# duylebkHCM/EyeDiseaseSegmentation

Measured on NVIDIA B200. Metric: IDRiD-size (2848x4288) fundus images/s, 4 lesion models, sliding-window + 8-view D4 TTA + AUC-PR, higher is better.
Workload: dtype bf16

## Files before the change

eyediseasesegmentation_b200/csrc/conv3x3_wide_sm100.cu:

```cuda
#include "tc_ptx.cuh"
#include <algorithm>
#include <cstdlib>
#include <cstring>
#include <mutex>

namespace eds {

constexpr int kWideThreads = 320;
constexpr int kWideStagesMax = 4;
constexpr int kWideRows = 8, kWideSlabCols = 32, kWideOutCols = 30, kWideSlabRows = kWideRows + 2;

struct WideParams {
    CUtensorMap a_map;
    CUtensorMap a_map1;
    int k_split;
    CUtensorMap b_map;
    CUtensorMap y_map;
    const float* bias;
    const __nv_bfloat16* residual;
    __nv_bfloat16* y;
    int C, block_k, k_chunks, bn;
    int N, H, W, relu;
    int tiles_w, tiles_h, total_tiles;
    int stages, atom_bytes, a_slab_bytes, b_box_bytes, stage_bytes, tmem_cols;
    int b_resident, b_region_bytes;
    int staged, staging_off;
    uint32_t idesc, desc_hi;
};

__device__ __forceinline__ void wide_mbar_arrive(uint64_t* bar) {
    asm volatile("mbarrier.arrive.shared::cta.b64 _, [%0];" ::"r"(smem_u32(bar)) : "memory");
}

__global__ void __launch_bounds__(kWideThreads, 1)
conv3x3_wide_kernel(const __grid_constant__ WideParams p) {
    extern __shared__ uint8_t smem_raw[];
    uint8_t* smem = reinterpret_cast<uint8_t*>((reinterpret_cast<uintptr_t>(smem_raw) + 1023) & ~(uintptr_t)1023);
    uint8_t* ring = smem + p.b_region_bytes;
    uint64_t* full_bar = reinterpret_cast<uint64_t*>(ring + (size_t)p.stages * p.stage_bytes);
    uint64_t* empty_bar = full_bar + kWideStagesMax;
    uint64_t* tmem_full_bar = empty_bar + kWideStagesMax;
    uint64_t* tmem_empty_bar = tmem_full_bar + 2;
    uint64_t* b_bar = tmem_empty_bar + 2;
    uint32_t* tmem_slot = reinterpret_cast<uint32_t*>(b_bar + 1);
    float* s_bias = reinterpret_cast<float*>(full_bar + 16);
    if (threadIdx.x < (unsigned)p.bn) s_bias[threadIdx.x] = p.bias ? __ldg(p.bias + threadIdx.x) : 0.f;

    const int warp = threadIdx.x >> 5, lane = threadIdx.x & 31;
    if (warp == 0 && lane == 0) {
        prefetch_tmap(&p.a_map);
        prefetch_tmap(&p.a_map1);
        prefetch_tmap(&p.b_map);
        for (int s = 0; s < p.stages; ++s) {
            mbar_init(&full_bar[s], 1);
            mbar_init(&empty_bar[s], 1);
        }
        for (int m = 0; m < 2; ++m) {
            mbar_init(&tmem_full_bar[m], 1);
            mbar_init(&tmem_empty_bar[m], 4);
        }
        mbar_init(b_bar, 1);
        asm volatile("fence.mbarrier_init.release.cluster;" ::: "memory");
        asm volatile("fence.proxy.async.shared::cta;" ::: "memory");
    }
    if (warp == 1) tmem_alloc(tmem_slot, (uint32_t)p.tmem_cols);
    tc_fence_before();
    __syncthreads();
    tc_fence_after();
    const uint32_t tmem_base = *tmem_slot;
    const uint32_t n3 = 3u * (uint32_t)p.bn;

    if (warp == 0) {
        if (lane == 0) {
            int stage = 0;
            uint32_t phase = 0;
            const uint32_t a_tx = (uint32_t)(kWideSlabRows * 4 * p.atom_bytes), b_tx = (uint32_t)(9 * p.bn * p.block_k * 2);
            const uint32_t tx = p.b_resident ? a_tx : a_tx + b_tx;
            if (p.b_resident) {
                mbar_arrive_expect_tx(b_bar, b_tx * (uint32_t)p.k_chunks);
                for (int kc = 0; kc < p.k_chunks; ++kc)
                    for (int tap = 0; tap < 9; ++tap)
                        tma_load_2d(smem + (size_t)(kc * 9 + tap) * p.b_box_bytes, &p.b_map, b_bar,
                                    tap * p.C + kc * p.block_k, 0);
            }
            for (int tile = blockIdx.x; tile < p.total_tiles; tile += gridDim.x) {
                const int tw = tile % p.tiles_w;
                const int t2 = tile / p.tiles_w;
                const int th = t2 % p.tiles_h;
                const int n = t2 / p.tiles_h;
                const int w0 = tw * kWideOutCols, h0 = th * kWideRows;
                for (int kc = 0; kc < p.k_chunks; ++kc) {
                    mbar_wait(&empty_bar[stage], phase ^ 1u);
                    mbar_arrive_expect_tx(&full_bar[stage], tx);
                    uint8_t* sa = ring + (size_t)stage * p.stage_bytes;
                    uint8_t* sb = sa + p.a_slab_bytes;
                    if (kc < p.k_split)
                        tma_load_4d(sa, &p.a_map, &full_bar[stage], kc * p.block_k, w0 - 1, h0 - 1, n);
                    else
                        tma_load_4d(sa, &p.a_map1, &full_bar[stage], (kc - p.k_split) * p.block_k, w0 - 1, h0 - 1, n);
                    if (!p.b_resident)
                        for (int tap = 0; tap < 9; ++tap)
                            tma_load_2d(sb + tap * p.b_box_bytes, &p.b_map, &full_bar[stage], tap * p.C + kc * p.block_k, 0);
                    if (++stage == p.stages) { stage = 0; phase ^= 1u; }
                }
            }
        }
    } else if (warp == 1) {
        int stage = 0;
        uint32_t phase = 0;
        const uint32_t lo0 = desc_lo(smem_u32(ring)), blo0 = desc_lo(smem_u32(smem));
        const uint32_t stage16 = (uint32_t)p.stage_bytes >> 4, slab16 = (uint32_t)p.a_slab_bytes >> 4;
        const uint32_t bchunk16 = 9u * ((uint32_t)p.b_box_bytes >> 4);
        if (p.b_resident) mbar_wait(b_bar, 0);
        const uint32_t atom16 = (uint32_t)p.atom_bytes >> 4, brow16 = 3u * ((uint32_t)p.b_box_bytes >> 4);
        const uint32_t dhi_w = p.desc_hi, idesc = p.idesc;
        const int k_steps = p.block_k / 16;
        int t = 0;
        for (int tile = blockIdx.x; tile < p.total_tiles; tile += gridDim.x, ++t) {
            const uint32_t empty_parity = (uint32_t)((t & 1) ^ 1);
            for (int kc = 0; kc < p.k_chunks; ++kc) {
                mbar_wait(&full_bar[stage], phase);
                const uint32_t a_st = lo0 + (uint32_t)stage * stage16;
                const uint32_t b_st = p.b_resident ? blo0 + (uint32_t)kc * bchunk16 : a_st + slab16;
#pragma unroll
                for (int m = 0; m < 2; ++m) {
                    if (kc == 0) mbar_wait(&tmem_empty_bar[m], empty_parity);
                    tc_fence_after();
                    if (elect_one()) {
                        const uint32_t d = tmem_base + (uint32_t)m * n3;
#pragma unroll
                        for (int dhi = 0; dhi < 3; ++dhi) {
                            const uint32_t a_lo = a_st + (uint32_t)(m * 16 + dhi * 4) * atom16;
                            const uint32_t b_lo = b_st + (uint32_t)dhi * brow16;
                            for (int ks = 0; ks < k_steps; ++ks)
                                umma_bf16_lohi(d, a_lo + 2u * ks, b_lo + 2u * ks, dhi_w, idesc,
                                               (kc > 0 || dhi > 0 || ks > 0) ? 1u : 0u);
                        }
                    }
                    __syncwarp();
                    if (kc == p.k_chunks - 1) {
                        if (elect_one()) umma_commit(&tmem_full_bar[m]);
                        __syncwarp();
                    }
                }
                if (elect_one()) umma_commit(&empty_bar[stage]);
                __syncwarp();
                if (++stage == p.stages) { stage = 0; phase ^= 1u; }
            }
        }
    } else {
        const int q = warp & 3;
        const int m = (warp - 2) >> 2;
        const int bn = p.bn;
        uint8_t* stg = smem + p.staging_off + (size_t)(warp - 2) * 4096;
        const int pos = lane - 1;
        int t = 0;
        for (int tile = blockIdx.x; tile < p.total_tiles; tile += gridDim.x, ++t) {
            const int tw = tile % p.tiles_w;
            const int t2 = tile / p.tiles_w;
            const int th = t2 % p.tiles_h;
            const int n = t2 / p.tiles_h;
            const int ow = tw * kWideOutCols - 1 + lane;
            const bool col_ok = lane >= 1 && lane <= kWideOutCols && ow < p.W;
            {
                mbar_wait(&tmem_full_bar[m], (uint32_t)(t & 1));
                tc_fence_after();
                const int oh = th * kWideRows + m * 4 + q;
                const bool valid = col_ok && oh < p.H;
                const int64_t off = (((int64_t)n * p.H + oh) * p.W + ow) * bn;
                const uint32_t taddr = tmem_base + ((uint32_t)(q * 32) << 16) + (uint32_t)m * n3;
                if (p.staged) {
                    if (lane == 0) asm volatile("cp.async.bulk.wait_group.read 0;" ::: "memory");
                    __syncwarp();
                }
                for (int c = 0; c < bn; c += 16) {
                    uint32_t rl[16], rc[16], rr[16];
                    tmem_ld16_nowait(taddr + (uint32_t)c, rl);
                    tmem_ld16_nowait(taddr + (uint32_t)(bn + c), rc);
                    tmem_ld16_nowait(taddr + (uint32_t)(2 * bn + c), rr);
                    tmem_ld_wait();
                    float v[16];
#pragma unroll
                    for (int i = 0; i < 16; ++i) {
                        const float l = __shfl_up_sync(0xffffffffu, __uint_as_float(rl[i]), 1);
                        const float r = __shfl_down_sync(0xffffffffu, __uint_as_float(rr[i]), 1);
                        v[i] = (l + __uint_as_float(rc[i])) + r;
                    }
                    if (valid || (p.staged && pos >= 0 && pos < kWideOutCols)) {
                        {
                            const float4* b4 = reinterpret_cast<const float4*>(s_bias + c);
#pragma unroll
                            for (int i = 0; i < 4; ++i) {
                                const float4 b = b4[i];
                                v[4 * i] += b.x; v[4 * i + 1] += b.y; v[4 * i + 2] += b.z; v[4 * i + 3] += b.w;
                            }
                        }
                        if (p.residual && valid) {
                            float r0[8], r1[8];
                            Vec8<__nv_bfloat16>::ld(p.residual + off + c, r0);
                            Vec8<__nv_bfloat16>::ld(p.residual + off + c + 8, r1);
#pragma unroll
                            for (int i = 0; i < 8; ++i) { v[i] += r0[i]; v[8 + i] += r1[i]; }
                        }
                        if (p.relu) {
#pragma unroll
                            for (int i = 0; i < 16; ++i) v[i] = fmaxf(v[i], 0.f);
                        }
                        float o0[8], o1[8];
#pragma unroll
                        for (int i = 0; i < 8; ++i) { o0[i] = v[i]; o1[i] = v[8 + i]; }
                        if (p.staged) {
                            const uint32_t j = (uint32_t)c >> 3, sw = (uint32_t)pos & 7u;
                            Vec8<__nv_bfloat16>::st(reinterpret_cast<__nv_bfloat16*>(stg + pos * 128 + ((j ^ sw) << 4)), o0);
                            Vec8<__nv_bfloat16>::st(reinterpret_cast<__nv_bfloat16*>(stg + pos * 128 + (((j + 1) ^ sw) << 4)), o1);
                        } else {
                            Vec8<__nv_bfloat16>::st(p.y + off + c, o0);
                            Vec8<__nv_bfloat16>::st(p.y + off + c + 8, o1);
                        }
                    }
                }
                if (p.staged) {
                    asm volatile("fence.proxy.async.shared::cta;" ::: "memory");
                    __syncwarp();
                    if (lane == 0 && oh < p.H) {
                        asm volatile(
                            "cp.async.bulk.tensor.4d.global.shared::cta.bulk_group [%0, {%2, %3, %4, %5}], [%1];"
                            ::"l"(&p.y_map), "r"(smem_u32(stg)), "r"(0), "r"(tw * kWideOutCols), "r"(oh), "r"(n)
                            : "memory");
                        asm volatile("cp.async.bulk.commit_group;" ::: "memory");
                    }
                }
                tc_fence_before();
                __syncwarp();
                if (lane == 0) wide_mbar_arrive(&tmem_empty_bar[m]);
            }
        }
        if (p.staged && lane == 0) asm volatile("cp.async.bulk.wait_group 0;" ::: "memory");
    }

    tc_fence_before();
    __syncthreads();
    if (warp == 1) tmem_dealloc(tmem_base, (uint32_t)p.tmem_cols);
}

static PerDevice g_wide_once;
static int g_wide_sms = 148;

static int wide_init() {
    return g_wide_once.run([](int dev) {
        cudaError_t e = cudaFuncSetAttribute(conv3x3_wide_kernel, cudaFuncAttributeMaxDynamicSharedMemorySize, 227 * 1024);
        if (e != cudaSuccess) {
            set_error("conv3x3_wide: cannot opt in to 227 KB shared memory: %s", cudaGetErrorString(e));
            return (int)EDS_ERR_CUDA;
        }
        int sms = 0;
        if (cudaDeviceGetAttribute(&sms, cudaDevAttrMultiProcessorCount, dev) == cudaSuccess && sms > 0) g_wide_sms = sms;
        return (int)EDS_OK;
    });
}

}

using namespace eds;

extern "C" int eds_conv3x3_wide_supported(int C, int Cout, int R, int S, int stride, int pad) {
    return R == 3 && S == 3 && stride == 1 && pad == 1 && C >= 16 && C % 16 == 0 && Cout >= 16 && Cout % 16 == 0 &&
           Cout <= 64;
}

static int wide_launch(const void* x, int C0, const void* x1, int C1, int N, int H, int W, const void* w,
                       const float* bias, int Cout, int relu, const void* residual, void* y, void* stream) {
    const int C = C0 + C1;
    EDS_REQUIRE(x && w && y, "conv3x3_wide: null pointer");
    EDS_REQUIRE(C0 >= 16 && C0 % 16 == 0 && C1 >= 0 && C1 % 16 == 0 && (x1 != nullptr) == (C1 > 0),
                "conv3x3_wide: C0=%d C1=%d must be multiples of 16", C0, C1);
    EDS_REQUIRE(N > 0 && H > 0 && W > 0, "conv3x3_wide: bad shape N=%d H=%d W=%d", N, H, W);
    EDS_REQUIRE(eds_conv3x3_wide_supported(C, Cout, 3, 3, 1, 1),
                "conv3x3_wide: C=%d Cout=%d outside the supported range (multiples of 16, Cout <= 64)", C, Cout);
    EDS_REQUIRE((((uintptr_t)x | (uintptr_t)x1 | (uintptr_t)w | (uintptr_t)y | (uintptr_t)residual | (uintptr_t)bias) &
                 15) == 0, "conv3x3_wide: pointers must be 16-byte aligned");
    if (int rc = igemm_init()) return rc;
    if (int rc = wide_init()) return rc;

    WideParams p;
    memset(&p, 0, sizeof(p));
    p.bias = bias;
    p.residual = (const __nv_bfloat16*)residual;
    p.y = (__nv_bfloat16*)y;
    p.C = C;
    p.block_k = ((C0 | C1) % 64 == 0) ? 64 : ((C0 | C1) % 32 == 0 ? 32 : 16);
    if (const char* bk = getenv("EDS_WIDE_BK")) {
        const int v = atoi(bk);
        if ((v == 32 || v == 16) && (C0 | C1) % v == 0) p.block_k = std::min(p.block_k, v);
    }
    p.k_chunks = C / p.block_k;
    p.k_split = C0 / p.block_k;
    p.bn = Cout;
    p.N = N; p.H = H; p.W = W; p.relu = relu;
    p.tiles_w = ceil_div(W, kWideOutCols);
    p.tiles_h = ceil_div(H, kWideRows);
    const int64_t total = (int64_t)p.tiles_w * p.tiles_h * N;
    EDS_REQUIRE(total < (1ll << 31), "conv3x3_wide: too many tiles");
    p.total_tiles = (int)total;

    const CUtensorMapSwizzle swz = p.block_k == 64 ? CU_TENSOR_MAP_SWIZZLE_128B
                                  : p.block_k == 32 ? CU_TENSOR_MAP_SWIZZLE_64B : CU_TENSOR_MAP_SWIZZLE_32B;
    const uint32_t layout = p.block_k == 64 ? 2u : (p.block_k == 32 ? 4u : 6u);
    p.atom_bytes = 8 * p.block_k * 2;
    const uint32_t sbo = (uint32_t)p.atom_bytes >> 4;
    p.desc_hi = sbo | (1u << 14) | (layout << 29);
    p.idesc = (1u << 4) | (1u << 7) | (1u << 10) | ((uint32_t)((3 * p.bn) >> 3) << 17) | ((uint32_t)(128 >> 4) << 24);
    p.a_slab_bytes = (kWideSlabRows * 4 * p.atom_bytes + 1023) & ~1023;
    p.b_box_bytes = p.bn * p.block_k * 2;
    const int barrier_bytes = 128 + 64 * 4;
    const int budget = 227 * 1024 - 1024 - barrier_bytes;
    const int b_all = p.k_chunks * 9 * p.b_box_bytes;
    static const bool no_resident = getenv("EDS_WIDE_RESIDENT") && atoi(getenv("EDS_WIDE_RESIDENT")) == 0;
    p.b_resident = !no_resident && b_all + 3 * p.a_slab_bytes <= budget;
    p.b_region_bytes = p.b_resident ? ((b_all + 1023) & ~1023) : 0;
    p.stage_bytes = p.b_resident ? p.a_slab_bytes : ((p.a_slab_bytes + 9 * p.b_box_bytes + 1023) & ~1023);
    p.stages = std::min(kWideStagesMax, (budget - p.b_region_bytes) / p.stage_bytes);
    EDS_REQUIRE(p.stages >= 2, "conv3x3_wide: a stage of %d B leaves no room for double buffering", p.stage_bytes);
    int cols = 32;
    while (cols < 6 * p.bn) cols <<= 1;
    p.tmem_cols = cols;
    static const bool no_staging = getenv("EDS_WIDE_STAGED") && atoi(getenv("EDS_WIDE_STAGED")) == 0;
    const int after_bars = p.b_region_bytes + p.stages * p.stage_bytes + barrier_bytes;
    p.staging_off = (after_bars + 1023) & ~1023;
    p.staged = !no_staging && p.bn == 64 && p.block_k == 64 && p.staging_off + 8 * 4096 + 1024 <= 227 * 1024;
    const size_t smem = (p.staged ? (size_t)p.staging_off + 8 * 4096 : (size_t)after_bars) + 1024;
    EDS_REQUIRE(smem <= 227 * 1024 && p.tmem_cols <= 512, "conv3x3_wide: tile does not fit (smem %zu, tmem %d)", smem,
                p.tmem_cols);

    {
        cuuint64_t dims[4] = {(cuuint64_t)C0, (cuuint64_t)W, (cuuint64_t)H, (cuuint64_t)N};
        cuuint64_t strides[3] = {(cuuint64_t)C0 * 2, (cuuint64_t)W * C0 * 2, (cuuint64_t)H * W * C0 * 2};
        cuuint32_t box[4] = {(cuuint32_t)p.block_k, (cuuint32_t)kWideSlabCols, (cuuint32_t)kWideSlabRows, 1u};
        if (int rc = tmap_encode_bf16(&p.a_map, x, 4, dims, strides, box, swz, "wide input")) return rc;
        p.a_map1 = p.a_map;
    }
    if (x1) {
        cuuint64_t dims[4] = {(cuuint64_t)C1, (cuuint64_t)W, (cuuint64_t)H, (cuuint64_t)N};
        cuuint64_t strides[3] = {(cuuint64_t)C1 * 2, (cuuint64_t)W * C1 * 2, (cuuint64_t)H * W * C1 * 2};
        cuuint32_t box[4] = {(cuuint32_t)p.block_k, (cuuint32_t)kWideSlabCols, (cuuint32_t)kWideSlabRows, 1u};
        if (int rc = tmap_encode_bf16(&p.a_map1, x1, 4, dims, strides, box, swz, "wide second input")) return rc;
    }
    {
        cuuint64_t dims[2] = {(cuuint64_t)9 * C, (cuuint64_t)Cout};
        cuuint64_t strides[1] = {(cuuint64_t)9 * C * 2};
        cuuint32_t box[2] = {(cuuint32_t)p.block_k, (cuuint32_t)p.bn};
        if (int rc = tmap_encode_bf16(&p.b_map, w, 2, dims, strides, box, swz, "wide weights")) return rc;
    }
    if (p.staged) {
        cuuint64_t dims[4] = {(cuuint64_t)Cout, (cuuint64_t)W, (cuuint64_t)H, (cuuint64_t)N};
        cuuint64_t strides[3] = {(cuuint64_t)Cout * 2, (cuuint64_t)W * Cout * 2, (cuuint64_t)H * W * Cout * 2};
        cuuint32_t box[4] = {64u, (cuuint32_t)kWideOutCols, 1u, 1u};
        if (int rc = tmap_encode_bf16(&p.y_map, y, 4, dims, strides, box, CU_TENSOR_MAP_SWIZZLE_128B, "wide output")) return rc;
    }
    const int grid = (int)std::min<int64_t>(total, g_wide_sms);
    conv3x3_wide_kernel<<<grid, kWideThreads, smem, as_stream(stream)>>>(p);
    return check_launch("conv3x3_wide_kernel");
}

extern "C" int eds_conv3x3_wide_bf16(const void* x, int N, int H, int W, int C, const void* w, const float* bias,
                                     int Cout, int relu, const void* residual, void* y, void* stream) {
    return wide_launch(x, C, nullptr, 0, N, H, W, w, bias, Cout, relu, residual, y, stream);
}

extern "C" int eds_conv3x3_wide_bf16_2src(const void* x0, int C0, const void* x1, int C1, int N, int H, int W,
                                          const void* w, const float* bias, int Cout, int relu, const void* residual,
                                          void* y, void* stream) {
    EDS_REQUIRE(x1 && C1 > 0, "conv3x3_wide_2src: second input missing");
    return wide_launch(x0, C0, x1, C1, N, H, W, w, bias, Cout, relu, residual, y, stream);
}
```

eyediseasesegmentation_b200/csrc/tc_ptx.cuh:

```cuda
#pragma once
#include "common.cuh"
#include <cuda.h>

namespace eds {

__device__ __forceinline__ uint32_t smem_u32(const void* p) { return (uint32_t)__cvta_generic_to_shared(p); }

__device__ __forceinline__ void mbar_init(uint64_t* bar, uint32_t count) {
    asm volatile("mbarrier.init.shared::cta.b64 [%0], %1;" ::"r"(smem_u32(bar)), "r"(count) : "memory");
}
__device__ __forceinline__ void mbar_arrive_expect_tx(uint64_t* bar, uint32_t bytes) {
    asm volatile("mbarrier.arrive.expect_tx.shared::cta.b64 _, [%0], %1;" ::"r"(smem_u32(bar)), "r"(bytes)
                 : "memory");
}
__device__ __forceinline__ bool mbar_try_wait(uint64_t* bar, uint32_t parity) {
    uint32_t ok;
    asm volatile(
        "{\n\t.reg .pred p;\n\t"
        "mbarrier.try_wait.parity.shared::cta.b64 p, [%1], %2;\n\t"
        "selp.u32 %0, 1, 0, p;\n\t}"
        : "=r"(ok)
        : "r"(smem_u32(bar)), "r"(parity)
        : "memory");
    return ok != 0;
}
__device__ __forceinline__ void mbar_wait(uint64_t* bar, uint32_t parity) {
    if (mbar_try_wait(bar, parity)) return;
    const long long t0 = clock64();
    while (!mbar_try_wait(bar, parity)) {
        if (clock64() - t0 > 4000000000LL) {
            printf("eds conv_igemm: mbarrier timeout (block %d thread %d)\n", (int)blockIdx.x, (int)threadIdx.x);
            __trap();
        }
    }
}
__device__ __forceinline__ void tma_load_4d(void* dst, const CUtensorMap* map, uint64_t* bar, int c0, int c1, int c2,
                                            int c3) {
    asm volatile(
        "cp.async.bulk.tensor.4d.shared::cluster.global.mbarrier::complete_tx::bytes [%0], [%1, {%3, %4, %5, %6}], [%2];"
        ::"r"(smem_u32(dst)), "l"(map), "r"(smem_u32(bar)), "r"(c0), "r"(c1), "r"(c2), "r"(c3)
        : "memory");
}
__device__ __forceinline__ void tma_load_2d(void* dst, const CUtensorMap* map, uint64_t* bar, int c0, int c1) {
    asm volatile(
        "cp.async.bulk.tensor.2d.shared::cluster.global.mbarrier::complete_tx::bytes [%0], [%1, {%3, %4}], [%2];"
        ::"r"(smem_u32(dst)), "l"(map), "r"(smem_u32(bar)), "r"(c0), "r"(c1)
        : "memory");
}
__device__ __forceinline__ void prefetch_tmap(const CUtensorMap* map) {
    asm volatile("prefetch.tensormap [%0];" ::"l"(map) : "memory");
}
__device__ __forceinline__ void tc_fence_before() { asm volatile("tcgen05.fence::before_thread_sync;" ::: "memory"); }
__device__ __forceinline__ void tc_fence_after() { asm volatile("tcgen05.fence::after_thread_sync;" ::: "memory"); }
__device__ __forceinline__ void tmem_alloc(uint32_t* dst, uint32_t cols) {
    asm volatile("tcgen05.alloc.cta_group::1.sync.aligned.shared::cta.b32 [%0], %1;" ::"r"(smem_u32(dst)), "r"(cols)
                 : "memory");
    asm volatile("tcgen05.relinquish_alloc_permit.cta_group::1.sync.aligned;" ::: "memory");
}
__device__ __forceinline__ void tmem_dealloc(uint32_t addr, uint32_t cols) {
    asm volatile("tcgen05.dealloc.cta_group::1.sync.aligned.b32 %0, %1;" ::"r"(addr), "r"(cols) : "memory");
}
__device__ __forceinline__ void umma_bf16(uint32_t tmem_d, uint64_t desc_a, uint64_t desc_b, uint32_t idesc,
                                          uint32_t accumulate) {
    asm volatile(
        "{\n\t.reg .pred p;\n\t"
        "setp.ne.b32 p, %4, 0;\n\t"
        "tcgen05.mma.cta_group::1.kind::f16 [%0], %1, %2, %3, p;\n\t}"
        ::"r"(tmem_d), "l"(desc_a), "l"(desc_b), "r"(idesc), "r"(accumulate)
        : "memory");
}
__device__ __forceinline__ void umma_commit(uint64_t* bar) {
    asm volatile("tcgen05.commit.cta_group::1.mbarrier::arrive::one.shared::cluster.b64 [%0];" ::"r"(smem_u32(bar))
                 : "memory");
}
__device__ __forceinline__ void tmem_ld16(uint32_t taddr, uint32_t (&r)[16]) {
    asm volatile(
        "tcgen05.ld.sync.aligned.32x32b.x16.b32 "
        "{%0, %1, %2, %3, %4, %5, %6, %7, %8, %9, %10, %11, %12, %13, %14, %15}, [%16];"
        : "=r"(r[0]), "=r"(r[1]), "=r"(r[2]), "=r"(r[3]), "=r"(r[4]), "=r"(r[5]), "=r"(r[6]), "=r"(r[7]), "=r"(r[8]),
          "=r"(r[9]), "=r"(r[10]), "=r"(r[11]), "=r"(r[12]), "=r"(r[13]), "=r"(r[14]), "=r"(r[15])
        : "r"(taddr)
        : "memory");
    asm volatile("tcgen05.wait::ld.sync.aligned;" ::: "memory");
}

__device__ __forceinline__ void tmem_ld16_nowait(uint32_t taddr, uint32_t (&r)[16]) {
    asm volatile(
        "tcgen05.ld.sync.aligned.32x32b.x16.b32 "
        "{%0, %1, %2, %3, %4, %5, %6, %7, %8, %9, %10, %11, %12, %13, %14, %15}, [%16];"
        : "=r"(r[0]), "=r"(r[1]), "=r"(r[2]), "=r"(r[3]), "=r"(r[4]), "=r"(r[5]), "=r"(r[6]), "=r"(r[7]), "=r"(r[8]),
          "=r"(r[9]), "=r"(r[10]), "=r"(r[11]), "=r"(r[12]), "=r"(r[13]), "=r"(r[14]), "=r"(r[15])
        : "r"(taddr)
        : "memory");
}
__device__ __forceinline__ void tmem_ld_wait() { asm volatile("tcgen05.wait::ld.sync.aligned;" ::: "memory"); }

__device__ __forceinline__ bool elect_one() {
    uint32_t pred;
    asm volatile(
        "{\n\t.reg .pred p;\n\t"
        "elect.sync _|p, 0xffffffff;\n\t"
        "selp.u32 %0, 1, 0, p;\n\t}"
        : "=r"(pred));
    return pred != 0;
}
__device__ __forceinline__ void umma_bf16_lohi(uint32_t tmem_d, uint32_t a_lo, uint32_t b_lo, uint32_t desc_hi,
                                               uint32_t idesc, uint32_t accumulate) {
    asm volatile(
        "{\n\t.reg .pred p;\n\t.reg .b64 da, db;\n\t"
        "setp.ne.b32 p, %5, 0;\n\t"
        "mov.b64 da, {%1, %3};\n\t"
        "mov.b64 db, {%2, %3};\n\t"
        "tcgen05.mma.cta_group::1.kind::f16 [%0], da, db, %4, p;\n\t}"
        ::"r"(tmem_d), "r"(a_lo), "r"(b_lo), "r"(desc_hi), "r"(idesc), "r"(accumulate)
        : "memory");
}
__device__ __forceinline__ uint32_t desc_lo(uint32_t saddr) { return ((saddr & 0x3FFFFu) >> 4) | (1u << 16); }

__device__ __forceinline__ uint64_t make_desc(uint32_t saddr, uint32_t desc_hi) {
    return (uint64_t)(((saddr & 0x3FFFFu) >> 4) | (1u << 16)) | ((uint64_t)desc_hi << 32);
}


int tmap_encode_bf16(CUtensorMap* map, const void* base, int rank, const cuuint64_t* dims, const cuuint64_t* strides,
                     const cuuint32_t* box, CUtensorMapSwizzle swz, const char* what);
int igemm_init();

}
```

Measured before the change: 1.859.

## Eliminate halo overlap in wide conv3x3 by carrying edge partials across tiles in TMEM

Each wide conv tile now loads 32 input columns with no horizontal halo, so tiles no longer overlap and no input columns are recomputed. The left and right partial sums that cross a tile boundary are kept in a TMEM carry region and added in by the next tile in the same row. Work is now assigned as contiguous tile ranges per CTA rather than strided, so carries stay within one CTA, and each range starts one tile early to rebuild its carry. In exchange the kernel needs more TMEM columns, does extra TMEM stores and loads, adds a special path for the last column, and releases the accumulator before the epilogue stores.

```diff
diff --git a/eyediseasesegmentation_b200/csrc/conv3x3_wide_sm100.cu b/eyediseasesegmentation_b200/csrc/conv3x3_wide_sm100.cu
--- a/eyediseasesegmentation_b200/csrc/conv3x3_wide_sm100.cu
+++ b/eyediseasesegmentation_b200/csrc/conv3x3_wide_sm100.cu
@@ -8,7 +8,7 @@
 
 constexpr int kWideThreads = 320;
 constexpr int kWideStagesMax = 4;
-constexpr int kWideRows = 8, kWideSlabCols = 32, kWideOutCols = 30, kWideSlabRows = kWideRows + 2;
+constexpr int kWideRows = 8, kWideCols = 32, kWideSlabRows = kWideRows + 2;
 
 struct WideParams {
     CUtensorMap a_map;
@@ -21,7 +21,7 @@
     __nv_bfloat16* y;
     int C, block_k, k_chunks, bn;
     int N, H, W, relu;
-    int tiles_w, tiles_h, total_tiles;
+    int tiles_w, bands, total_tiles;
     int stages, atom_bytes, a_slab_bytes, b_box_bytes, stage_bytes, tmem_cols;
     int b_resident, b_region_bytes;
     int staged, staging_off;
@@ -30,6 +30,48 @@
 
 __device__ __forceinline__ void wide_mbar_arrive(uint64_t* bar) {
     asm volatile("mbarrier.arrive.shared::cta.b64 _, [%0];" ::"r"(smem_u32(bar)) : "memory");
+}
+
+__device__ __forceinline__ void wide_store16(const WideParams& p, const float* s_bias, uint8_t* stg, const float* acc,
+                                             int c, int pos, bool valid, int64_t off) {
+    if (!stg && !valid) return;
+    float v[16];
+    const float4* b4 = reinterpret_cast<const float4*>(s_bias + c);
+#pragma unroll
+    for (int i = 0; i < 4; ++i) {
+        const float4 b = b4[i];
+        v[4 * i] = acc[4 * i] + b.x; v[4 * i + 1] = acc[4 * i + 1] + b.y;
+        v[4 * i + 2] = acc[4 * i + 2] + b.z; v[4 * i + 3] = acc[4 * i + 3] + b.w;
+    }
+    if (p.residual && valid) {
+        float r0[8], r1[8];
+        Vec8<__nv_bfloat16>::ld(p.residual + off + c, r0);
+        Vec8<__nv_bfloat16>::ld(p.residual + off + c + 8, r1);
+#pragma unroll
+        for (int i = 0; i < 8; ++i) { v[i] += r0[i]; v[8 + i] += r1[i]; }
+    }
+    if (p.relu) {
+#pragma unroll
+        for (int i = 0; i < 16; ++i) v[i] = fmaxf(v[i], 0.f);
+    }
+    float o0[8], o1[8];
+#pragma unroll
+    for (int i = 0; i < 8; ++i) { o0[i] = v[i]; o1[i] = v[8 + i]; }
+    if (stg) {
+        const uint32_t j = (uint32_t)c >> 3, sw = (uint32_t)pos & 7u;
+        Vec8<__nv_bfloat16>::st(reinterpret_cast<__nv_bfloat16*>(stg + pos * 128 + ((j ^ sw) << 4)), o0);
+        Vec8<__nv_bfloat16>::st(reinterpret_cast<__nv_bfloat16*>(stg + pos * 128 + (((j + 1) ^ sw) << 4)), o1);
+    } else {
+        Vec8<__nv_bfloat16>::st(p.y + off + c, o0);
+        Vec8<__nv_bfloat16>::st(p.y + off + c + 8, o1);
+    }
+}
+
+__device__ __forceinline__ void wide_tile_range(const WideParams& p, int* first, int* emit, int* end) {
+    const int64_t total = p.total_tiles;
+    *emit = (int)(total * blockIdx.x / gridDim.x);
+    *end = (int)(total * (blockIdx.x + 1) / gridDim.x);
+    *first = *emit - (*emit % p.tiles_w != 0 ? 1 : 0);
 }
 
 __global__ void __launch_bounds__(kWideThreads, 1)
@@ -83,25 +125,28 @@
                         tma_load_2d(smem + (size_t)(kc * 9 + tap) * p.b_box_bytes, &p.b_map, b_bar,
                                     tap * p.C + kc * p.block_k, 0);
             }
-            for (int tile = blockIdx.x; tile < p.total_tiles; tile += gridDim.x) {
-                const int tw = tile % p.tiles_w;
-                const int t2 = tile / p.tiles_w;
-                const int th = t2 % p.tiles_h;
-                const int n = t2 / p.tiles_h;
-                const int w0 = tw * kWideOutCols, h0 = th * kWideRows;
-                for (int kc = 0; kc < p.k_chunks; ++kc) {
-                    mbar_wait(&empty_bar[stage], phase ^ 1u);
-                    mbar_arrive_expect_tx(&full_bar[stage], tx);
-                    uint8_t* sa = ring + (size_t)stage * p.stage_bytes;
-                    uint8_t* sb = sa + p.a_slab_bytes;
-                    if (kc < p.k_split)
-                        tma_load_4d(sa, &p.a_map, &full_bar[stage], kc * p.block_k, w0 - 1, h0 - 1, n);
-                    else
-                        tma_load_4d(sa, &p.a_map1, &full_bar[stage], (kc - p.k_split) * p.block_k, w0 - 1, h0 - 1, n);
-                    if (!p.b_resident)
-                        for (int tap = 0; tap < 9; ++tap)
-                            tma_load_2d(sb + tap * p.b_box_bytes, &p.b_map, &full_bar[stage], tap * p.C + kc * p.block_k, 0);
-                    if (++stage == p.stages) { stage = 0; phase ^= 1u; }
+            int first, emit, end;
+            wide_tile_range(p, &first, &emit, &end);
+            for (int u = first; u < end; ++u) {
+                const int strip = u / p.tiles_w;
+                const int n = strip / p.bands, h0 = (strip % p.bands) * kWideRows;
+                {
+                    const int w0 = (u % p.tiles_w) * kWideCols;
+                    for (int kc = 0; kc < p.k_chunks; ++kc) {
+                        mbar_wait(&empty_bar[stage], phase ^ 1u);
+                        mbar_arrive_expect_tx(&full_bar[stage], tx);
+                        uint8_t* sa = ring + (size_t)stage * p.stage_bytes;
+                        uint8_t* sb = sa + p.a_slab_bytes;
+                        if (kc < p.k_split)
+                            tma_load_4d(sa, &p.a_map, &full_bar[stage], kc * p.block_k, w0, h0 - 1, n);
+                        else
+                            tma_load_4d(sa, &p.a_map1, &full_bar[stage], (kc - p.k_split) * p.block_k, w0, h0 - 1, n);
+                        if (!p.b_resident)
+                            for (int tap = 0; tap < 9; ++tap)
+                                tma_load_2d(sb + tap * p.b_box_bytes, &p.b_map, &full_bar[stage], tap * p.C + kc * p.block_k,
+                                            0);
+                        if (++stage == p.stages) { stage = 0; phase ^= 1u; }
+                    }
                 }
             }
         }
@@ -115,8 +160,9 @@
         const uint32_t atom16 = (uint32_t)p.atom_bytes >> 4, brow16 = 3u * ((uint32_t)p.b_box_bytes >> 4);
         const uint32_t dhi_w = p.desc_hi, idesc = p.idesc;
         const int k_steps = p.block_k / 16;
-        int t = 0;
-        for (int tile = blockIdx.x; tile < p.total_tiles; tile += gridDim.x, ++t) {
+        int first, emit, end;
+        wide_tile_range(p, &first, &emit, &end);
+        for (int t = 0; t < end - first; ++t) {
             const uint32_t empty_parity = (uint32_t)((t & 1) ^ 1);
             for (int kc = 0; kc < p.k_chunks; ++kc) {
                 mbar_wait(&full_bar[stage], phase);
@@ -152,87 +198,79 @@
         const int q = warp & 3;
         const int m = (warp - 2) >> 2;
         const int bn = p.bn;
-        uint8_t* stg = smem + p.staging_off + (size_t)(warp - 2) * 4096;
-        const int pos = lane - 1;
-        int t = 0;
-        for (int tile = blockIdx.x; tile < p.total_tiles; tile += gridDim.x, ++t) {
-            const int tw = tile % p.tiles_w;
-            const int t2 = tile / p.tiles_w;
-            const int th = t2 % p.tiles_h;
-            const int n = t2 / p.tiles_h;
-            const int ow = tw * kWideOutCols - 1 + lane;
-            const bool col_ok = lane >= 1 && lane <= kWideOutCols && ow < p.W;
+        uint8_t* stg = !p.staged || lane == 31 ? nullptr : smem + p.staging_off + (size_t)(warp - 2) * 4096;
+        const int src_l = (lane + 31) & 31, src_r = (lane + 1) & 31;
+        const uint32_t taddr = tmem_base + ((uint32_t)(q * 32) << 16) + (uint32_t)m * n3;
+        const uint32_t tcarry = tmem_base + ((uint32_t)(q * 32) << 16) + 2u * n3 + (uint32_t)(m * bn);
+        int first, emit, end;
+        wide_tile_range(p, &first, &emit, &end);
+        for (int u = first, t = 0; u < end; ++u, ++t) {
+            const int strip = u / p.tiles_w, tw = u % p.tiles_w;
+            const int n = strip / p.bands;
+            const int oh = (strip % p.bands) * kWideRows + m * 4 + q;
+            const bool row_out = u >= emit && oh < p.H;
             {
+                const int ow = tw * kWideCols + (lane == 31 ? -1 : lane);
+                const bool valid = row_out && ow >= 0 && ow < p.W;
+                const int64_t off = (((int64_t)n * p.H + oh) * p.W + ow) * bn;
                 mbar_wait(&tmem_full_bar[m], (uint32_t)(t & 1));
                 tc_fence_after();
-                const int oh = th * kWideRows + m * 4 + q;
-                const bool valid = col_ok && oh < p.H;
-                const int64_t off = (((int64_t)n * p.H + oh) * p.W + ow) * bn;
-                const uint32_t taddr = tmem_base + ((uint32_t)(q * 32) << 16) + (uint32_t)m * n3;
+                float v[64];
+#pragma unroll
+                for (int g = 0; g < 8; ++g) {
+                    if (g * 8 >= bn) break;
+                    const int c = g * 8;
+                    uint32_t rl[8], rc[8], rr[8], rk[8];
+                    tmem_ld8_nowait(taddr + (uint32_t)c, rl);
+                    tmem_ld8_nowait(taddr + (uint32_t)(bn + c), rc);
+                    tmem_ld8_nowait(taddr + (uint32_t)(2 * bn + c), rr);
+                    tmem_ld8_nowait(tcarry + (uint32_t)c, rk);
+                    tmem_ld_wait();
+#pragma unroll
+                    for (int i = 0; i < 8; ++i) {
+                        const float l = __shfl_sync(0xffffffffu, __uint_as_float(rl[i]), src_l);
+                        const float r = __shfl_sync(0xffffffffu, __uint_as_float(rr[i]), src_r);
+                        const float k = tw == 0 ? 0.f : __uint_as_float(rk[i]);
+                        const float part = (lane == 0 ? k : l) + __uint_as_float(rc[i]);
+                        v[c + i] = (lane == 31 ? k : part) + r;
+                        rk[i] = __float_as_uint(lane == 0 ? l : part);
+                    }
+                    tmem_st8(tcarry + (uint32_t)c, rk);
+                }
+                tmem_st_wait();
+                tc_fence_before();
+                __syncwarp();
+                if (lane == 0) wide_mbar_arrive(&tmem_empty_bar[m]);
                 if (p.staged) {
                     if (lane == 0) asm volatile("cp.async.bulk.wait_group.read 0;" ::: "memory");
                     __syncwarp();
                 }
-                for (int c = 0; c < bn; c += 16) {
-                    uint32_t rl[16], rc[16], rr[16];
-                    tmem_ld16_nowait(taddr + (uint32_t)c, rl);
-                    tmem_ld16_nowait(taddr + (uint32_t)(bn + c), rc);
-                    tmem_ld16_nowait(taddr + (uint32_t)(2 * bn + c), rr);
-                    tmem_ld_wait();
-                    float v[16];
-#pragma unroll
-                    for (int i = 0; i < 16; ++i) {
-                        const float l = __shfl_up_sync(0xffffffffu, __uint_as_float(rl[i]), 1);
-                        const float r = __shfl_down_sync(0xffffffffu, __uint_as_float(rr[i]), 1);
-                        v[i] = (l + __uint_as_float(rc[i])) + r;
-                    }
-                    if (valid || (p.staged && pos >= 0 && pos < kWideOutCols)) {
-                        {
-                            const float4* b4 = reinterpret_cast<const float4*>(s_bias + c);
-#pragma unroll
-                            for (int i = 0; i < 4; ++i) {
-                                const float4 b = b4[i];
-                                v[4 * i] += b.x; v[4 * i + 1] += b.y; v[4 * i + 2] += b.z; v[4 * i + 3] += b.w;
-                            }
-                        }
-                        if (p.residual && valid) {
-                            float r0[8], r1[8];
-                            Vec8<__nv_bfloat16>::ld(p.residual + off + c, r0);
-                            Vec8<__nv_bfloat16>::ld(p.residual + off + c + 8, r1);
-#pragma unroll
-                            for (int i = 0; i < 8; ++i) { v[i] += r0[i]; v[8 + i] += r1[i]; }
-                        }
-                        if (p.relu) {
-#pragma unroll
-                            for (int i = 0; i < 16; ++i) v[i] = fmaxf(v[i], 0.f);
-                        }
-                        float o0[8], o1[8];
-#pragma unroll
-                        for (int i = 0; i < 8; ++i) { o0[i] = v[i]; o1[i] = v[8 + i]; }
-                        if (p.staged) {
-                            const uint32_t j = (uint32_t)c >> 3, sw = (uint32_t)pos & 7u;
-                            Vec8<__nv_bfloat16>::st(reinterpret_cast<__nv_bfloat16*>(stg + pos * 128 + ((j ^ sw) << 4)), o0);
-                            Vec8<__nv_bfloat16>::st(reinterpret_cast<__nv_bfloat16*>(stg + pos * 128 + (((j + 1) ^ sw) << 4)), o1);
-                        } else {
-                            Vec8<__nv_bfloat16>::st(p.y + off + c, o0);
-                            Vec8<__nv_bfloat16>::st(p.y + off + c + 8, o1);
-                        }
+#pragma unroll
+                for (int g = 0; g < 4; ++g)
+                    if (g * 16 < bn) wide_store16(p, s_bias, stg, v + g * 16, g * 16, lane, valid, off);
+                if (tw == p.tiles_w - 1 && (p.W & 31) == 0 && row_out) {
+#pragma unroll
+                    for (int g = 0; g < 4; ++g) {
+                        if (g * 16 >= bn) break;
+                        uint32_t rk[16];
+                        tmem_ld16(tcarry + (uint32_t)(g * 16), rk);
+                        float f[16];
+#pragma unroll
+                        for (int i = 0; i < 16; ++i) f[i] = __fadd_rn(__uint_as_float(rk[i]), 0.f);
+                        if (lane == 31) wide_store16(p, s_bias, nullptr, f, g * 16, 0, true, off + 32 * bn);
                     }
                 }
                 if (p.staged) {
                     asm volatile("fence.proxy.async.shared::cta;" ::: "memory");
                     __syncwarp();
-                    if (lane == 0 && oh < p.H) {
+                    if (lane == 0 && row_out) {
                         asm volatile(
                             "cp.async.bulk.tensor.4d.global.shared::cta.bulk_group [%0, {%2, %3, %4, %5}], [%1];"
-                            ::"l"(&p.y_map), "r"(smem_u32(stg)), "r"(0), "r"(tw * kWideOutCols), "r"(oh), "r"(n)
+                            ::"l"(&p.y_map), "r"(smem_u32(stg)), "r"(0), "r"(tw * kWideCols), "r"(oh), "r"(n)
                             : "memory");
                         asm volatile("cp.async.bulk.commit_group;" ::: "memory");
                     }
                 }
-                tc_fence_before();
-                __syncwarp();
-                if (lane == 0) wide_mbar_arrive(&tmem_empty_bar[m]);
             }
         }
         if (p.staged && lane == 0) asm volatile("cp.async.bulk.wait_group 0;" ::: "memory");
@@ -297,9 +335,9 @@
     p.k_split = C0 / p.block_k;
     p.bn = Cout;
     p.N = N; p.H = H; p.W = W; p.relu = relu;
-    p.tiles_w = ceil_div(W, kWideOutCols);
-    p.tiles_h = ceil_div(H, kWideRows);
-    const int64_t total = (int64_t)p.tiles_w * p.tiles_h * N;
+    p.tiles_w = ceil_div(W, kWideCols);
+    p.bands = ceil_div(H, kWideRows);
+    const int64_t total = (int64_t)p.bands * N * p.tiles_w;
     EDS_REQUIRE(total < (1ll << 31), "conv3x3_wide: too many tiles");
     p.total_tiles = (int)total;
 
@@ -322,7 +360,7 @@
     p.stages = std::min(kWideStagesMax, (budget - p.b_region_bytes) / p.stage_bytes);
     EDS_REQUIRE(p.stages >= 2, "conv3x3_wide: a stage of %d B leaves no room for double buffering", p.stage_bytes);
     int cols = 32;
-    while (cols < 6 * p.bn) cols <<= 1;
+    while (cols < 8 * p.bn) cols <<= 1;
     p.tmem_cols = cols;
     static const bool no_staging = getenv("EDS_WIDE_STAGED") && atoi(getenv("EDS_WIDE_STAGED")) == 0;
     const int after_bars = p.b_region_bytes + p.stages * p.stage_bytes + barrier_bytes;
@@ -335,14 +373,14 @@
     {
         cuuint64_t dims[4] = {(cuuint64_t)C0, (cuuint64_t)W, (cuuint64_t)H, (cuuint64_t)N};
         cuuint64_t strides[3] = {(cuuint64_t)C0 * 2, (cuuint64_t)W * C0 * 2, (cuuint64_t)H * W * C0 * 2};
-        cuuint32_t box[4] = {(cuuint32_t)p.block_k, (cuuint32_t)kWideSlabCols, (cuuint32_t)kWideSlabRows, 1u};
+        cuuint32_t box[4] = {(cuuint32_t)p.block_k, (cuuint32_t)kWideCols, (cuuint32_t)kWideSlabRows, 1u};
         if (int rc = tmap_encode_bf16(&p.a_map, x, 4, dims, strides, box, swz, "wide input")) return rc;
         p.a_map1 = p.a_map;
     }
     if (x1) {
         cuuint64_t dims[4] = {(cuuint64_t)C1, (cuuint64_t)W, (cuuint64_t)H, (cuuint64_t)N};
         cuuint64_t strides[3] = {(cuuint64_t)C1 * 2, (cuuint64_t)W * C1 * 2, (cuuint64_t)H * W * C1 * 2};
-        cuuint32_t box[4] = {(cuuint32_t)p.block_k, (cuuint32_t)kWideSlabCols, (cuuint32_t)kWideSlabRows, 1u};
+        cuuint32_t box[4] = {(cuuint32_t)p.block_k, (cuuint32_t)kWideCols, (cuuint32_t)kWideSlabRows, 1u};
         if (int rc = tmap_encode_bf16(&p.a_map1, x1, 4, dims, strides, box, swz, "wide second input")) return rc;
     }
     {
@@ -354,7 +392,7 @@
     if (p.staged) {
         cuuint64_t dims[4] = {(cuuint64_t)Cout, (cuuint64_t)W, (cuuint64_t)H, (cuuint64_t)N};
         cuuint64_t strides[3] = {(cuuint64_t)Cout * 2, (cuuint64_t)W * Cout * 2, (cuuint64_t)H * W * Cout * 2};
-        cuuint32_t box[4] = {64u, (cuuint32_t)kWideOutCols, 1u, 1u};
+        cuuint32_t box[4] = {64u, (cuuint32_t)kWideCols - 1, 1u, 1u};
         if (int rc = tmap_encode_bf16(&p.y_map, y, 4, dims, strides, box, CU_TENSOR_MAP_SWIZZLE_128B, "wide output")) return rc;
     }
     const int grid = (int)std::min<int64_t>(total, g_wide_sms);
diff --git a/eyediseasesegmentation_b200/csrc/tc_ptx.cuh b/eyediseasesegmentation_b200/csrc/tc_ptx.cuh
--- a/eyediseasesegmentation_b200/csrc/tc_ptx.cuh
+++ b/eyediseasesegmentation_b200/csrc/tc_ptx.cuh
@@ -94,6 +94,18 @@
         : "memory");
 }
 __device__ __forceinline__ void tmem_ld_wait() { asm volatile("tcgen05.wait::ld.sync.aligned;" ::: "memory"); }
+__device__ __forceinline__ void tmem_ld8_nowait(uint32_t taddr, uint32_t (&r)[8]) {
+    asm volatile("tcgen05.ld.sync.aligned.32x32b.x8.b32 {%0, %1, %2, %3, %4, %5, %6, %7}, [%8];"
+                 : "=r"(r[0]), "=r"(r[1]), "=r"(r[2]), "=r"(r[3]), "=r"(r[4]), "=r"(r[5]), "=r"(r[6]), "=r"(r[7])
+                 : "r"(taddr)
+                 : "memory");
+}
+__device__ __forceinline__ void tmem_st8(uint32_t taddr, const uint32_t (&r)[8]) {
+    asm volatile("tcgen05.st.sync.aligned.32x32b.x8.b32 [%0], {%1, %2, %3, %4, %5, %6, %7, %8};"
+                 ::"r"(taddr), "r"(r[0]), "r"(r[1]), "r"(r[2]), "r"(r[3]), "r"(r[4]), "r"(r[5]), "r"(r[6]), "r"(r[7])
+                 : "memory");
+}
+__device__ __forceinline__ void tmem_st_wait() { asm volatile("tcgen05.wait::st.sync.aligned;" ::: "memory"); }
 
 __device__ __forceinline__ bool elect_one() {
     uint32_t pred;
```

New measurement: 1.878 (median of 6 runs). 1.01x the previous value.
